# PrinceVictor/LWSNet

Measured on AMD Instinct MI355X. Metric: stereo pairs/sec @256x512 maxdisp=192 (stage-4), higher is better.
Workload: dtype f32; 1 GPU; BASELINE config 2: batch=1/GPU, 256x512 synthetic pair, maxdisplist=[24,5,5], all 4 stages; pairs_per_gpu=1, streams=1, parallelism=single GPU, weights=seeded synthetic (seed 7, calibrated BN), GPU_MAX_HW_QUEUES=4

## Files before the change

lwsnet_amd/csrc/lws_api.hip:

```cpp
#include <math.h>
#include <stdarg.h>
#include <stdio.h>
#include <string.h>

#include <algorithm>
#include <stdlib.h>

#include "lws_common.h"

namespace lws {

static thread_local char g_err[512] = "";
thread_local hipEvent_t tl_stop_event = nullptr;

void set_error(const char *fmt, ...)
{
    va_list ap;
    va_start(ap, fmt);
    vsnprintf(g_err, sizeof(g_err), fmt, ap);
    va_end(ap);
}

typedef std::map<std::string, std::vector<int64_t>> Spec;

// ... 701 lines not shown
                      "maxdisplist[%d] must be in 1..32 (got %d)", i, cfg->maxdisplist[i]);
    for (int i = 0; i < 3; ++i) {
        const int c3 = cfg->channels_3d * cfg->growth_rate[i];
        LWS_CHECK_ARG(c3 == 8 || c3 == 16 || c3 == 32,
                      "stage %d: channels_3d*growth_rate = %d is not supported by the gfx950 kernels (8, 16, 32)", i, c3);
    }
    LWS_CHECK_ARG(cfg->feature_fp16 == 0 || cfg->feature_fp16 == 1, "feature_fp16 must be 0 or 1 (got %d)", cfg->feature_fp16);
    LWS_CHECK_ARG(cfg->interp_align_mode == 0 || cfg->interp_align_mode == 1, "interp_align_mode must be 0 or 1 (got %d)",
                  cfg->interp_align_mode);
    lws_ctx *h = new (std::nothrow) lws_ctx();
    if (!h) {
        set_error("out of host memory");
        return LWS_ERR_NOMEM;
    }
    h->cfg = *cfg;
    h->spec = build_spec(*cfg);
    for (int i = 0; i < 3; ++i) h->stage[i].c3 = cfg->channels_3d * cfg->growth_rate[i];
    if (hipGetDevice(&h->device) != hipSuccess) h->device = -1;
    (void)hipGetLastError();
    *out = h;
    return LWS_OK;
}

static void apply_options(lws_ctx *h)
{
    for (int i = 0; i < 3; ++i) {
        h->stage[i].mid16_split = (h->opt.split_bf16 & 1) != 0;
        h->stage[i].mid8_split = (h->opt.split_bf16 & 2) != 0;
        h->stage[i].mid8_balance = h->mid8_balance;
        h->stage[i].cu_count = h->cu_count;
    }
    h->net2d.r2_first.form = (h->opt.split_bf16 & 4) ? 1 : 0;
}

static int *option_slot(lws_ctx *h, const char *name)
{
    struct { const char *name; int *slot; } tab[] = {{"fuse_first", &h->opt.fuse_first},
                                                     {"defer_upsample", &h->opt.defer_upsample},
                                                     {"side_streams", &h->opt.side_streams},
                                                     {"split_bf16", &h->opt.split_bf16},
                                                     {"ref_chunk_mb", &h->opt.ref_chunk_mb},
                                                     {"ref_pipe", &h->opt.ref_pipe},
                                                     {"warp_form", &h->opt.warp_form},
                                                     {"fuse_last1", &h->opt.fuse_last1},
                                                     {"fork2_after", &h->opt.fork2_after},
                                                     {"fuse_ref_last", &h->opt.fuse_ref_last},
                                                     {"device", &h->device}};
    for (auto &e : tab)
        if (strcmp(e.name, name) == 0) return e.slot;
    return nullptr;
}

int lws_set_option(lws_handle h, const char *name, int value)
{
    LWS_CHECK_ARG(h && name, "lws_set_option: null argument");
    int *slot = option_slot(h, name);
    LWS_CHECK_ARG(slot != nullptr, "lws_set_option: unknown option '%s'", name);
    if (strcmp(name, "split_bf16") == 0)
        LWS_CHECK_ARG(value >= 0 && value <= 7, "lws_set_option: split_bf16 is a bit mask in 0..7 (got %d)", value);
    else if (strcmp(name, "fuse_first") == 0)
        LWS_CHECK_ARG(value >= 0 && value <= 3, "lws_set_option: fuse_first is a bit mask in 0..3 (got %d)", value);
    else if (strcmp(name, "ref_pipe") == 0 || strcmp(name, "fuse_ref_last") == 0)
        LWS_CHECK_ARG(value >= -1 && value <= 1, "lws_set_option: %s is out of range (got %d)", name, value);
    else if (strcmp(name, "ref_chunk_mb") == 0)
        LWS_CHECK_ARG(value >= 0 && value <= 4096, "lws_set_option: ref_chunk_mb must be in 0..4096 (got %d)", value);
    else if (strcmp(name, "device") == 0) {
        LWS_CHECK_ARG(value >= 0, "lws_set_option: device must be >= 0 (got %d)", value);
        LWS_CHECK_ARG(h->params == nullptr && h->ws == nullptr && h->side == nullptr,
                      "lws_set_option: the device of a handle can only be changed before lws_finalize / lws_reserve "
                      "have allocated on device %d", h->device);
    }
    else if (strcmp(name, "fork2_after") == 0)
        LWS_CHECK_ARG(value >= -1 && value <= 16, "lws_set_option: fork2_after must be in -1..16 (got %d)", value);
    else
        LWS_CHECK_ARG(value == 0 || value == 1, "lws_set_option: %s must be 0 or 1 (got %d)", name, value);
    *slot = value;
    apply_options(h);
    return LWS_OK;
}

int lws_get_option(lws_handle h, const char *name, int *value)
{
    LWS_CHECK_ARG(h && name && value, "lws_get_option: null argument");
    int *slot = option_slot(h, name);
    LWS_CHECK_ARG(slot != nullptr, "lws_get_option: unknown option '%s'", name);
    *value = *slot;
    return LWS_OK;
}

int lws_profile_enable(lws_handle h, int class_mask)
{
    LWS_CHECK_ARG(h, "lws_profile_enable: null handle");
    prof_clear(h);
    h->prof_mask = h->prof_mask_cfg = (unsigned)class_mask;
    h->prof_every = 1;
    h->prof_calls = 0;
    return LWS_OK;
}

int lws_profile_sample(lws_handle h, int every_n)
{
    LWS_CHECK_ARG(h && every_n >= 1, "lws_profile_sample: every_n must be >= 1");
    h->prof_every = every_n;
    h->prof_calls = 0;
    return LWS_OK;
}

int lws_profile_read(lws_handle h, double *total_ms, int64_t *launches)
{
    LWS_CHECK_ARG(h && total_ms && launches, "lws_profile_read: null argument");
    LWS_CHECK_DEVICE(h, "lws_profile_read");
    for (int i = 0; i < LWS_KC_COUNT; ++i) {
        total_ms[i] = 0.0;
        launches[i] = 0;
    }
    for (lws_prof_rec &r : h->prof) {
        LWS_HIP(hipEventSynchronize(r.t1));
        float ms = 0.f;
        LWS_HIP(hipEventElapsedTime(&ms, r.t0, r.t1));
        total_ms[r.kc] += ms;
        launches[r.kc] += 1;
    }
    return LWS_OK;
}

int lws_profile_read_class(lws_handle h, int kernel_class, float *ms_out, int capacity, int *count)
{
    LWS_CHECK_ARG(h && count && (ms_out || capacity == 0) && capacity >= 0, "lws_profile_read_class: bad argument");
    LWS_CHECK_ARG(kernel_class >= 0 && kernel_class < LWS_KC_COUNT, "lws_profile_read_class: unknown kernel class %d", kernel_class);
    LWS_CHECK_DEVICE(h, "lws_profile_read_class");
    int n = 0;
    for (lws_prof_rec &r : h->prof) {
        if (r.kc != kernel_class) continue;
        if (n < capacity) {
            LWS_HIP(hipEventSynchronize(r.t1));
            float ms = 0.f;
            LWS_HIP(hipEventElapsedTime(&ms, r.t0, r.t1));
            ms_out[n] = ms;
        }
        ++n;
    }
    *count = n;
    return LWS_OK;
}

int lws_clock_stamp(lws_handle h, int enable)
{
    LWS_CHECK_ARG(h, "lws_clock_stamp: null handle");
    LWS_CHECK_DEVICE(h, "lws_clock_stamp");
    if (enable) {
        if (h->stage[0].c3 == 8) {
            set_error("lws_clock_stamp: stage 1 of this model has C3 = 8: no k_conv3d_mid16 launch to stamp");
            return LWS_ERR_STATE;
        }
        if (!h->clk_buf) LWS_HIP(hipMalloc(&h->clk_buf, kClockWgs * 4 * sizeof(unsigned long long)));
        LWS_HIP(hipMemset(h->clk_buf, 0, kClockWgs * 4 * sizeof(unsigned long long)));
    }
    h->stage[0].clk = enable ? h->clk_buf : nullptr;
    return LWS_OK;
}

int lws_clock_read(lws_handle h, double *ghz)
{
    LWS_CHECK_ARG(h && ghz, "lws_clock_read: null argument");
    LWS_CHECK_DEVICE(h, "lws_clock_read");
    if (!h->clk_buf) {
// ... 351 lines not shown
```

lwsnet_amd/csrc/lws_common.h:

```cpp
#pragma once
#include <hip/hip_runtime.h>
#include <hip/hip_ext.h>
#include <stdint.h>

#include <atomic>
#include <map>
#include <string>
#include <vector>

#include "lwsnet_hip.h"

namespace lws {

void set_error(const char *fmt, ...) __attribute__((format(printf, 1, 2)));

#define LWS_CHECK_ARG(cond, ...)                 \
    do {                                         \
        if (!(cond)) {                           \
            ::lws::set_error(__VA_ARGS__);       \
            return LWS_ERR_INVALID;              \
        }                                        \
    } while (0)

#define LWS_HIP(call)                                                                           \
// ... 169 lines not shown
struct lws_ctx {
    lws_config cfg;
    struct {
        int fuse_first = 3;
        int defer_upsample = 1;
        int side_streams = 1;
        int split_bf16 = 0;
        int ref_pipe = -1;
        int warp_form = 1;
        int fuse_last1 = 1;
        int fork2_after = -1;
        int fuse_ref_last = -1;
        int ref_chunk_mb = 72;
    } opt;
    unsigned prof_mask = 0;
    unsigned prof_mask_cfg = 0;
    int prof_every = 1;
    unsigned prof_calls = 0;
    std::vector<lws_prof_rec> prof;
    std::vector<hipEvent_t> evt_pool;
    int device = 0;
    int cu_count = 0;
    bool finalized = false;
    std::map<std::string, std::vector<float>> host;
    std::map<std::string, std::vector<int64_t>> shapes;
    std::map<std::string, std::vector<int64_t>> spec;
    float *params = nullptr;
    bool owns_params = true;
    size_t params_bytes = 0;
    lws::Stage3d stage[3];
    lws::Net2d net2d;
    bool have_2d = false;
    float *ws = nullptr;
    size_t ws_bytes = 0;
    int mid8_balance = 1;
    hipStream_t side = nullptr;
    hipEvent_t ev_fork = nullptr, ev_join = nullptr;
    hipEvent_t ev_feat[3] = {nullptr, nullptr, nullptr};
    hipEvent_t ev_fork2 = nullptr;
    unsigned long long *clk_buf = nullptr;
};

namespace lws {

struct StageMap {
    float *mem = nullptr;
    bool written = false;
    const float *low = nullptr;
    int h = 0, w = 0;
    StageMap *prev = nullptr;
};
int check_stage_map(const StageMap &m, bool nested, const char *who);

int launch_volume_l1_shift(const float *L, const float *R, float *cost, int B, int C, int h, int w, int D,
                           hipStream_t st, bool q16 = false);
int launch_volume_l1_warp(const float *L, const float *R, StageMap &prev, float *cost, float *wflow_out,
                          int B, int C, int h, int w, int H, int W, int m, hipStream_t st, bool q16 = false,
                          int form = 1,
                          float ioff = 0.5f);
int launch_softargmin(const float *cost, float *low, int B, int D, int h, int w, float start, hipStream_t st);
int launch_upsample_add(const float *low, const float *prev, float *out, int B, int h, int w, int H, int W,
                        hipStream_t st, float ioff = 0.5f);
int launch_softargmin_upsample(const float *cost, const float *prev, float *out, float *low_out, int B, int D, int h,
                               int w, int H, int W, float start, hipStream_t st, float ioff = 0.5f);

bool shift_first_can_fuse(const Stage3d &s, int C);
int launch_shift_first(const Stage3d &s, const float *L, const float *R, float *cost, float *act_out, int B, int C, int D,
                       int h, int w, hipStream_t st, bool q16);
int launch_conv3d_first(const Stage3d &s, const float *cost, float *act_out, int B, int D, int h, int w,
                        hipStream_t st);
int launch_conv3d_mid(const Stage3d &s, int layer, const float *act_in, float *act_out, int B, int D, int h,
                      int w, hipStream_t st, hipEvent_t e0 = nullptr, hipEvent_t e1 = nullptr);
int launch_conv3d_last(const Stage3d &s, const float *act_in, const float *cost_skip, float *cost_out, int B,
                       int D, int h, int w, hipStream_t st);

int launch_conv2d_nchw(const Conv2dLayer &l, const float *in, const float *res, float *out, int N, int H, int W,
                       hipStream_t st, const float *in2 = nullptr, int n1 = 0);
int conv2d_pair_groups(int layer);
void pack_pair_mfma(const float *w, int cin, float *out);
int launch_conv2d_pair(const Conv2dLayer &a, const Conv2dLayer &b, const float *in, const float *res, float *out, int N,
                       int H, int W, hipStream_t st, const float *in2 = nullptr, int n1 = 0);
int launch_ref_first(const float *in, int cin, const float *w, float *out, int B, int H, int W, hipStream_t st);
int launch_ref_dws(const RefDws &l, const float *in, float *out, int B, int H, int W, hipStream_t st);
bool ref_first_dws_can_fuse(const RefDws &l, int cin);
int launch_ref_first_dws(const RefDws &l, StageMap &in, int cin, const float *wfrag, float *out, int B, int H, int W,
                         hipStream_t st, float ioff = 0.5f);
int packed_first_mfma_floats(int cin);
void pack_first_mfma(const float *w , int cin, float *out);
int launch_ref_conv64(const RefConv64 &l, const float *inL, const float *inD, float *out, int B, int H, int W,
                      hipStream_t st);
int launch_ref_last(const float *in, const float *w, const float *pred3, float *out, int B, int H, int W, hipStream_t st);
bool ref_dws_last_can_fuse(const RefDws &l);
int launch_ref_dws_last(const RefDws &l, const float *in, const float *wlast, const float *pred3, float *out, int B, int H, int W,
                        hipStream_t st);
void pack_conv2d_mfma(const float *w, int cin, int ktaps, float *out);
size_t packed_conv64x_floats();
void pack_conv64_bf16x3(const float *w, float *out);

bool conv3d_last_can_fuse(const Stage3d &s, int D);
int launch_conv3d_last_softargmin(const Stage3d &s, const float *act_in, const float *cost_skip, float *cost_out,
                                  float *low, float start, int B, int D, int h, int w, hipStream_t st);

size_t packed_mid_weight_floats(int c3);
void pack_mid_weights(const float *w , int c3, float *out);
void pack_first8_weights(const float *w , float *out );
void pack_first16_weights(const float *w , int c3, float *out );

}
```

lwsnet_amd/csrc/lws_conv2d.hip:

```cpp
#include "lws_common.h"
#include "lws_device_math.h"

namespace lws {


LWS_DEFINE_STAMPS(conv2d)

__device__ __forceinline__ float bn_relu2(float x, float s, float t) { return fmaxf(fmaf(x, s, t), 0.0f); }
__device__ __forceinline__ float f4c(const float4 &v, int j) { return j == 0 ? v.x : j == 1 ? v.y : j == 2 ? v.z : v.w; }

template <int CIN, int COUT, bool TRANSPOSED>
__global__ __launch_bounds__(256) void k_conv2d_nchw(const float *__restrict__ in, const float *__restrict__ in2, int n1,
                                                     const float *__restrict__ wgt,
                                                     const float *__restrict__ bn_s, const float *__restrict__ bn_t,
                                                     const float *__restrict__ res, float *__restrict__ out, int H,
                                                     int W, int Ho, int Wo, int stride, int pad, int dil, int relu,
                                                     int RH, int RW, int RWp)
{
    constexpr int CPT = COUT / 4;
    extern __shared__ float sIn[];
    const int b = blockIdx.z;
    const int tid = threadIdx.x, tx = tid & 7, ty = (tid >> 3) & 7;
    const int wave_id = __builtin_amdgcn_readfirstlane(tid >> 6);
    const int co0 = wave_id * CPT;
// ... 420 lines not shown
}

int launch_conv2d_pair(const Conv2dLayer &a, const Conv2dLayer &b, const float *in, const float *res, float *out, int N,
                       int H, int W, hipStream_t st, const float *in2, int n1)
{
    if (a.transposed || b.transposed || b.stride != 1 || b.pad != b.dil || a.pad != a.dil || a.bn_s == nullptr ||
        b.cin != a.cout) {
        set_error("conv2d_pair: unsupported layer pair");
        return LWS_ERR_INVALID;
    }
    if (in2 == nullptr) {
        in2 = in;
        n1 = N;
    }
    const int HA = (H + 2 * a.pad - 2 * a.dil - 1) / a.stride + 1, WA = (W + 2 * a.pad - 2 * a.dil - 1) / a.stride + 1;
    if (a.cout == 16 && b.cout == 16 && a.stride == 2 && a.dil == 1 && b.dil == 1 && res == nullptr &&
        a.w_mfma != nullptr && b.w_mfma != nullptr && (a.cin == 8 || a.cin == 16)) {
        if (a.cin == 8) return conv2d_pair_mfma_launch<8>(a, b, in, in2, n1, out, N, H, W, HA, WA, st);
        return conv2d_pair_mfma_launch<16>(a, b, in, in2, n1, out, N, H, W, HA, WA, st);
    }
#define LWS_C2P(CI, CMID, CO, SA, DA, DB, NW)                                                             \
    if (a.cin == CI && a.cout == CMID && b.cout == CO && a.stride == SA && a.dil == DA && b.dil == DB)    \
        return conv2d_pair_launch<CI, CMID, CO, SA, DA, DB, NW>(a, b, in, in2, n1, res, out, N, H, W, HA, WA, st);
    LWS_C2P(3, 4, 8, 2, 2, 4, 4) LWS_C2P(8, 4, 8, 1, 2, 2, 4) LWS_C2P(8, 16, 16, 2, 1, 1, 16) LWS_C2P(16, 16, 16, 2, 1, 1, 16)
#undef LWS_C2P
    set_error("conv2d_pair: unsupported pair %d -> %d -> %d (stride %d, dilations %d, %d)", a.cin, a.cout, b.cout, a.stride,
              a.dil, b.dil);
    return LWS_ERR_INVALID;
}

template <int CIN>
__global__ __launch_bounds__(256) void k_ref_first(const float *__restrict__ in, const float *__restrict__ wgt,
                                                   float *__restrict__ out, int H, int W)
{
    __shared__ __attribute__((aligned(16))) float sW[9 * CIN * 32];
    for (int i = threadIdx.x; i < 9 * CIN * 32; i += 256) sW[i] = wgt[i];
    __syncthreads();
    const int64_t plane = (int64_t)H * W;
    const int64_t idx = (int64_t)blockIdx.x * 256 + threadIdx.x;
    const int64_t pix = idx >> 2;
    const int grp = (int)(idx & 3), b = blockIdx.y;
    if (pix >= plane) return;
    const int y = (int)(pix / W), x = (int)(pix % W);
    const float *inb = in + (int64_t)b * CIN * plane;
    float acc[8];
#pragma unroll
    for (int c = 0; c < 8; ++c) acc[c] = 0.0f;
#pragma unroll 3
    for (int tap = 0; tap < 9; ++tap) {
        const int kh = tap / 3, kw = tap - kh * 3;
        const int iy = y + kh - 1, ix = x + kw - 1;
        const bool ok = iy >= 0 && iy < H && ix >= 0 && ix < W;
#pragma unroll
        for (int ci = 0; ci < CIN; ++ci) {
            const float ld = inb[ok ? (int64_t)ci * plane + (int64_t)iy * W + ix : 0];
            const float v = ok ? ld : 0.0f;
            const float4 w0 = *reinterpret_cast<const float4 *>(&sW[(tap * CIN + ci) * 32 + grp * 8]);
            const float4 w1 = *reinterpret_cast<const float4 *>(&sW[(tap * CIN + ci) * 32 + grp * 8 + 4]);
            acc[0] = fmaf(v, w0.x, acc[0]);
            acc[1] = fmaf(v, w0.y, acc[1]);
            acc[2] = fmaf(v, w0.z, acc[2]);
            acc[3] = fmaf(v, w0.w, acc[3]);
            acc[4] = fmaf(v, w1.x, acc[4]);
            acc[5] = fmaf(v, w1.y, acc[5]);
            acc[6] = fmaf(v, w1.z, acc[6]);
            acc[7] = fmaf(v, w1.w, acc[7]);
        }
    }
    float4 *o = reinterpret_cast<float4 *>(out + ((int64_t)b * plane + pix) * 32 + grp * 8);
    o[0] = make_float4(acc[0], acc[1], acc[2], acc[3]);
    o[1] = make_float4(acc[4], acc[5], acc[6], acc[7]);
}

constexpr int RT_Y = 8, RT_X = 16;
constexpr int RH_Y = RT_Y + 2, RH_X = RT_X + 2;
constexpr int RVS = 32;

__device__ __forceinline__ int swz(int p, int grp) { return p * RVS + ((grp ^ (p & 7)) << 2); }

struct RefTile {
    int b, Y0, X0;
};

__device__ __forceinline__ RefTile ref_tile(int dil, int nbx, int nby, int tile_rows = RT_Y)
{
    int bid = blockIdx.x;
    const int d2 = dil * dil;
    const int phase = bid % d2;
    bid /= d2;
    const int bx = bid % nbx;
    bid /= nbx;
    const int by = bid % nby;
    RefTile t;
    t.b = bid / nby;
    t.Y0 = by * tile_rows * dil + phase / dil;
    t.X0 = bx * RT_X * dil + phase % dil;
    return t;
}

constexpr int DWS_SA = 186, DWS_SB = 130;

constexpr int DWS_FD = 2, DWS_FR = (RH_Y - 1) * DWS_FD + 3, DWS_FC = (RH_X - 1) * DWS_FD + 3;
static_assert(DWS_FR * DWS_FC <= 1024 && 3 * DWS_FR * DWS_FC <= 8 * DWS_SB * 4, "first-conv window must fit 4 loads/thread/plane and sB");

template <int CIN>
__device__ __forceinline__ void first_conv_mfma(const float *sImg, const float *__restrict__ wfrag,
                                                const float *__restrict__ bn_s, const float *__restrict__ bn_t, float4 *sA,
                                                int Y0, int X0, int H, int W, int lane, int wave)
{
    constexpr int WIN = DWS_FR * DWS_FC, K = 9 * CIN, J = (K + 3) / 4, NPX = RH_Y * RH_X, NTW = 3;
    static_assert(4 * NTW * 16 >= NPX, "three N-tiles per wave must cover the halo tile");
    const int n = lane & 15, g = lane >> 4;
    float a[2][J];
#pragma unroll
    for (int mt = 0; mt < 2; ++mt)
#pragma unroll
        for (int j = 0; j < J; ++j) a[mt][j] = wfrag[(mt * J + j) * 64 + lane];
    int koff[J];
#pragma unroll
    for (int j = 0; j < J; ++j) {
        const int k = 4 * j + g, tap = k / CIN, ci = k - tap * CIN, kh = tap / 3, kw = tap - kh * 3;
        koff[j] = k < K ? ci * WIN + kh * DWS_FC + kw : 0;
    }
    float4 s4[2], t4[2];
#pragma unroll
    for (int mt = 0; mt < 2; ++mt) {
        s4[mt] = *reinterpret_cast<const float4 *>(bn_s + (mt * 4 + g) * 4);
        t4[mt] = *reinterpret_cast<const float4 *>(bn_t + (mt * 4 + g) * 4);
    }
#pragma unroll
    for (int nt = 0; nt < NTW; ++nt) {
        const int hp = (wave * NTW + nt) * 16 + n;
        const int hy = hp / RH_X, hx = hp - hy * RH_X;
        const float *sp = sImg + (hp < NPX ? (hy * DWS_FD) * DWS_FC + hx * DWS_FD : 0);
        floatx4 acc[2] = {(floatx4){0.f, 0.f, 0.f, 0.f}, (floatx4){0.f, 0.f, 0.f, 0.f}};
#pragma unroll
        for (int j = 0; j < J; ++j) {
            const float b = sp[koff[j]];
#pragma unroll
            for (int mt = 0; mt < 2; ++mt) acc[mt] = __builtin_amdgcn_mfma_f32_16x16x4f32(a[mt][j], b, acc[mt], 0, 0, 0);
        }
        const int gy = Y0 + (hy - 1) * DWS_FD, gx = X0 + (hx - 1) * DWS_FD;
        const bool ok = hp < NPX && gy >= 0 && gy < H && gx >= 0 && gx < W;
#pragma unroll
        for (int mt = 0; mt < 2; ++mt) {
            float4 v = bn_relu4(make_float4(acc[mt][0], acc[mt][1], acc[mt][2], acc[mt][3]), s4[mt], t4[mt]);
            if (!ok) v = make_float4(0.f, 0.f, 0.f, 0.f);
            if (hp < NPX) sA[(mt * 4 + g) * DWS_SA + hp] = v;
        }
    }
}

template <int FIRST>
__global__ __launch_bounds__(256, 4) void k_ref_dws(const float *__restrict__ in, const float *__restrict__ wf,
                                                 const float *__restrict__ bn_s,
                                                 const float *__restrict__ bn_t, const float *dw,
                                                 const float4 *pwpk,
                                                 float *__restrict__ out, int H, int W, int dil, int nbx, int nby, int wt,
                                                 const float *__restrict__ plow, int ph, int pw, float *__restrict__ pmat,
                                                 float ioff)
{
    __shared__ float4 sA[8 * DWS_SA];
    __shared__ float4 sB[8 * DWS_SB];
    const int tid = threadIdx.x, lane = tid & 63, wave = tid >> 6;
    const RefTile t = ref_tile(dil, nbx, nby);
    LWS_STAMPK(5, 0);

    const int c4 = tid & 7;
    const float4 s4 = *reinterpret_cast<const float4 *>(bn_s + c4 * 4);
    const float4 t4 = *reinterpret_cast<const float4 *>(bn_t + c4 * 4);

    constexpr int NPX = RH_Y * RH_X, SITER = (NPX * 8 + 255) / 256;
    float4 c[SITER];
    bool okv[SITER];
    if (FIRST == 3) {
        float *sImg = reinterpret_cast<float *>(sB);
        constexpr int WIN = DWS_FR * DWS_FC, NLD = (3 * WIN + 255) / 256;
        const float *inb = in + (int64_t)t.b * 3 * H * W;
        const int gy0 = t.Y0 - DWS_FD - 1, gx0 = t.X0 - DWS_FD - 1;
        float iv[NLD];
#pragma unroll
        for (int k = 0; k < NLD; ++k) {
            const int r3 = tid + 256 * k;
            const int ci = r3 / WIN, r = r3 - ci * WIN;
            const int ry = r / DWS_FC, rx = r - ry * DWS_FC;
            const int gy = gy0 + ry, gx = gx0 + rx;
            const bool ok = r3 < 3 * WIN && gy >= 0 && gy < H && gx >= 0 && gx < W;
            const float ld = inb[ok ? (int64_t)ci * H * W + (int64_t)gy * W + gx : 0];
            iv[k] = ok ? ld : 0.0f;
        }
#pragma unroll
        for (int k = 0; k < NLD; ++k)
            if (tid + 256 * k < 3 * WIN) sImg[tid + 256 * k] = iv[k];
        __syncthreads();
        first_conv_mfma<3>(sImg, wf, bn_s, bn_t, sA, t.Y0, t.X0, H, W, lane, wave);
        __syncthreads();
    } else if (FIRST == 1) {
        float *sImg = reinterpret_cast<float *>(sB);
        DeferredMap dm{plow != nullptr ? plow + (int64_t)t.b * ph * pw : nullptr, in + (int64_t)t.b * H * W, ph, pw,
                       (float)H, 1.0f / (float)(ph > 0 ? ph : 1)};
        dm.off = ioff;
        const int gy0 = t.Y0 - DWS_FD - 1, gx0 = t.X0 - DWS_FD - 1;
        float iv[4];
        bool iok[4];
        int iys[4], ixs[4];
#pragma unroll
        for (int k = 0; k < 4; ++k) {
            const int r = tid + 256 * k;
            const int ry = r / DWS_FC, rx = r - ry * DWS_FC;
            const int gy = gy0 + ry, gx = gx0 + rx;
            iok[k] = r < DWS_FR * DWS_FC && gy >= 0 && gy < H && gx >= 0 && gx < W;
            iys[k] = iok[k] ? gy : 0;
            ixs[k] = iok[k] ? gx : 0;
        }
        deferred_at_n<4>(dm, iys, ixs, H, W, iv);
#pragma unroll
        for (int k = 0; k < 4; ++k)
            if (tid + 256 * k < DWS_FR * DWS_FC) sImg[tid + 256 * k] = iok[k] ? iv[k] : 0.0f;
        __syncthreads();
        if (pmat != nullptr && tid < RT_Y * RT_X) {
            const int ty = tid / RT_X, tx = tid - ty * RT_X;
            const int gy = t.Y0 + ty * DWS_FD, gx = t.X0 + tx * DWS_FD;
            if (gy < H && gx < W)
                pmat[(int64_t)t.b * H * W + (int64_t)gy * W + gx] = sImg[((ty + 1) * DWS_FD + 1) * DWS_FC + (tx + 1) * DWS_FD + 1];
        }
        first_conv_mfma<1>(sImg, wf, bn_s, bn_t, sA, t.Y0, t.X0, H, W, lane, wave);
        __syncthreads();
    } else {
        const float *inb = in + (int64_t)t.b * H * W * 32;
#pragma unroll
        for (int i = 0; i < SITER; ++i) {
            const int hp = (tid >> 3) + 32 * i;
            const int hy = hp / RH_X, hx = hp - hy * RH_X;
            const int gy = t.Y0 + (hy - 1) * dil, gx = t.X0 + (hx - 1) * dil;
            okv[i] = hp < NPX && gy >= 0 && gy < H && gx >= 0 && gx < W;
            const int off = okv[i] ? (gy * W + gx) * 32 + c4 * 4 : 0;
            c[i] = *reinterpret_cast<const float4 *>(inb + off);
        }
    }
    float4 aw[2][2];
#pragma unroll
    for (int q = 0; q < 2; ++q)
#pragma unroll
        for (int mt = 0; mt < 2; ++mt) aw[q][mt] = pwpk[(q * 2 + mt) * 64 + lane];
    float4 wd[9];
#pragma unroll
    for (int tap = 0; tap < 9; ++tap) wd[tap] = *reinterpret_cast<const float4 *>(dw + tap * 32 + c4 * 4);
    if (FIRST == 0) {
#pragma unroll
        for (int i = 0; i < SITER; ++i) {
            const int hp = (tid >> 3) + 32 * i;
            float4 v = bn_relu4(c[i], s4, t4);
            if (!okv[i]) v = make_float4(0.f, 0.f, 0.f, 0.f);
            if (hp < NPX) sA[c4 * DWS_SA + hp] = v;
        }
        __syncthreads();
    }
    LWS_STAMPK(5, 1);

    {
        const int q = c4 >> 2, a_ = c4 & 3;
        const int x = (tid >> 3) & 15, rg = tid >> 7;
        const float4 *src = sA + c4 * DWS_SA + (4 * rg) * RH_X + x;
        float4 acc[4];
#pragma unroll
        for (int j = 0; j < 4; ++j) acc[j] = make_float4(0.f, 0.f, 0.f, 0.f);
#pragma unroll
        for (int rr = 0; rr < 6; ++rr) {
            const float4 t0 = src[rr * RH_X], t1 = src[rr * RH_X + 1], t2 = src[rr * RH_X + 2];
#pragma unroll
            for (int j = 0; j < 4; ++j) {
                const int kh = rr - j;
                if (kh >= 0 && kh < 3) {
                    fma4(acc[j], t0, wd[kh * 3 + 0]);
                    fma4(acc[j], t1, wd[kh * 3 + 1]);
                    fma4(acc[j], t2, wd[kh * 3 + 2]);
                }
            }
        }
        float *dst = reinterpret_cast<float *>(sB + (4 * q) * DWS_SB + (4 * rg) * RT_X + x) + a_;
#pragma unroll
        for (int j = 0; j < 4; ++j) {
            dst[(0 * DWS_SB + RT_X * j) * 4] = acc[j].x;
            dst[(1 * DWS_SB + RT_X * j) * 4] = acc[j].y;
            dst[(2 * DWS_SB + RT_X * j) * 4] = acc[j].z;
            dst[(3 * DWS_SB + RT_X * j) * 4] = acc[j].w;
        }
    }
    __syncthreads();
    LWS_STAMPK(5, 2);

    const int n = lane & 15, g = lane >> 4;
    floatx4 acc[2][2];
#pragma unroll
    for (int r = 0; r < 2; ++r)
#pragma unroll
        for (int mt = 0; mt < 2; ++mt) acc[r][mt] = (floatx4){0.f, 0.f, 0.f, 0.f};
    float4 bv[2][2];
#pragma unroll
    for (int r = 0; r < 2; ++r)
#pragma unroll
        for (int q = 0; q < 2; ++q) bv[r][q] = sB[(4 * q + g) * DWS_SB + (2 * wave + r) * RT_X + n];
#pragma unroll
    for (int q = 0; q < 2; ++q)
#pragma unroll
        for (int j = 0; j < 4; ++j)
#pragma unroll
            for (int r = 0; r < 2; ++r)
#pragma unroll
                for (int mt = 0; mt < 2; ++mt)
                    acc[r][mt] = __builtin_amdgcn_mfma_f32_16x16x4f32(f4c(aw[q][mt], j), f4c(bv[r][q], j), acc[r][mt], 0, 0, 0);

    LWS_STAMPK(5, 3);
    float *outb = out + (int64_t)t.b * H * W * 32;
    const int gx = t.X0 + n * dil;
#pragma unroll
    for (int r = 0; r < 2; ++r) {
        const int gy = t.Y0 + (2 * wave + r) * dil;
        if (gy < H && gx < W) {
            float *o = outb + (gy * W + gx) * 32;
#pragma unroll
            for (int mt = 0; mt < 2; ++mt)
                store_act4(o + mt * 16 + 4 * g, make_float4(acc[r][mt][0], acc[r][mt][1], acc[r][mt][2], acc[r][mt][3]), wt);
        }
    }
}

template <int TY, int NW>
__global__ __launch_bounds__(64 * NW) void k_ref_conv64(const float *__restrict__ inL, const float *__restrict__ inD,
                                                    const float *__restrict__ bn_s, const float *__restrict__ bn_t,
                                                    const float4 *__restrict__ wpk,
                                                    float *__restrict__ out, int H, int W, int dil, int nbx, int nby, int wt)
{
    constexpr int HY = TY + 2, NPX = HY * RH_X, RW = TY / NW, NT = 64 * NW;
    static_assert(TY % NW == 0 && RW >= 1 && RW <= 4, "rows must split evenly over the waves");
    __shared__ __attribute__((aligned(16))) float sA[2 * NPX * RVS];
    const int tid = threadIdx.x, lane = tid & 63, wave = tid >> 6;
    const RefTile t = ref_tile(dil, nbx, nby, TY);
    const int n = lane & 15, g = lane >> 4;
    LWS_STAMPK(6, 0);

    constexpr int ITEMS = 2 * NPX * 2, SITER = (ITEMS + NT - 1) / NT;
    {
        float4 c[SITER][4];
        bool okv[SITER];
#pragma unroll
        for (int i = 0; i < SITER; ++i) {
            const int it = tid + i * NT;
            const int q = it & 1, hp = (it >> 1) % NPX, ten = (it >> 1) / NPX;
            const int hy = hp / RH_X, hx = hp % RH_X;
            const int gy = t.Y0 + (hy - 1) * dil, gx = t.X0 + (hx - 1) * dil;
            okv[i] = it < ITEMS && gy >= 0 && gy < H && gx >= 0 && gx < W;
            const float *base = (ten == 1 && it < ITEMS ? inD : inL) + (int64_t)t.b * H * W * 32;
            const float4 *src = reinterpret_cast<const float4 *>(base + (okv[i] ? ((int64_t)gy * W + gx) * 32 + q * 16 : 0));
#pragma unroll
            for (int k = 0; k < 4; ++k) c[i][k] = src[k];
        }
#pragma unroll
        for (int i = 0; i < SITER; ++i) {
            const int it = tid + i * NT;
            if (it < ITEMS) {
                const int q = it & 1, hp = (it >> 1) % NPX, ten = (it >> 1) / NPX;
                const float4 *sp = reinterpret_cast<const float4 *>(bn_s + ten * 32 + q * 16);
                const float4 *tp = reinterpret_cast<const float4 *>(bn_t + ten * 32 + q * 16);
                float4 a[4];
#pragma unroll
                for (int k = 0; k < 4; ++k) {
                    const float4 v = c[i][k], sc = sp[k], tt = tp[k];
                    a[k] = make_float4(bn_relu2(v.x, sc.x, tt.x), bn_relu2(v.y, sc.y, tt.y), bn_relu2(v.z, sc.z, tt.z),
                                       bn_relu2(v.w, sc.w, tt.w));
                    if (!okv[i]) a[k] = make_float4(0.f, 0.f, 0.f, 0.f);
                }
                float *img = sA + ten * NPX * RVS;
                *reinterpret_cast<float4 *>(&img[swz(hp, 4 * q + 0)]) = make_float4(a[0].x, a[1].x, a[2].x, a[3].x);
                *reinterpret_cast<float4 *>(&img[swz(hp, 4 * q + 1)]) = make_float4(a[0].y, a[1].y, a[2].y, a[3].y);
                *reinterpret_cast<float4 *>(&img[swz(hp, 4 * q + 2)]) = make_float4(a[0].z, a[1].z, a[2].z, a[3].z);
                *reinterpret_cast<float4 *>(&img[swz(hp, 4 * q + 3)]) = make_float4(a[0].w, a[1].w, a[2].w, a[3].w);
            }
        }
    }
    const float4 *wp = wpk + lane;
    float4 wbuf[2][4][2];
#pragma unroll
    for (int qq = 0; qq < 4; ++qq)
#pragma unroll
        for (int mt = 0; mt < 2; ++mt) wbuf[0][qq][mt] = wp[(qq * 2 + mt) * 64];
    __syncthreads();
    LWS_STAMPK(6, 1);

    floatx4 acc[RW][2];
#pragma unroll
    for (int r = 0; r < RW; ++r)
#pragma unroll
        for (int mt = 0; mt < 2; ++mt) acc[r][mt] = (floatx4){0.f, 0.f, 0.f, 0.f};
    auto frag = [&](int r, int tap, int qq) {
        const int hp = (RW * wave + r + tap / 3) * RH_X + n + tap % 3;
        return *reinterpret_cast<const float4 *>(&sA[(qq >> 1) * NPX * RVS + swz(hp, 4 * (qq & 1) + g)]);
    };
    float4 bbuf[2][RW];
#pragma unroll
    for (int r = 0; r < RW; ++r) bbuf[0][r] = frag(r, 0, 0);
#pragma unroll 1
    for (int tap = 0; tap < 9; ++tap) {
        const int tn = tap < 8 ? tap + 1 : 8;
#pragma unroll
        for (int qq = 0; qq < 4; ++qq) {
            float4 *bc = bbuf[qq & 1], *bn = bbuf[(qq & 1) ^ 1];
// ... 301 lines not shown
                dst[(2 * FL_SB) * 4] = acc.z;
                dst[(3 * FL_SB) * 4] = acc.w;
            }
        }
    }
    __syncthreads();

    {
        constexpr int NTW = FL_NT / 4;
        const int n = lane & 15, g = lane >> 4;
        floatx4 acc[NTW][2];
        float4 bv[NTW][2];
#pragma unroll
        for (int r = 0; r < NTW; ++r) {
#pragma unroll
            for (int mt = 0; mt < 2; ++mt) acc[r][mt] = (floatx4){0.f, 0.f, 0.f, 0.f};
#pragma unroll
            for (int q = 0; q < 2; ++q) bv[r][q] = sB[(4 * q + g) * FL_SB + (wave * NTW + r) * 16 + n];
        }
#pragma unroll
        for (int q = 0; q < 2; ++q)
#pragma unroll
            for (int j = 0; j < 4; ++j)
#pragma unroll
                for (int r = 0; r < NTW; ++r)
#pragma unroll
                    for (int mt = 0; mt < 2; ++mt)
                        acc[r][mt] = __builtin_amdgcn_mfma_f32_16x16x4f32(f4c(aw[q][mt], j), f4c(bv[r][q], j), acc[r][mt], 0, 0, 0);
#pragma unroll
        for (int r = 0; r < NTW; ++r) {
            const int p = (wave * NTW + r) * 16 + n;
            if (p < FL_NM) {
                const int my = p / FL_MX, mx = p - my * FL_MX;
                const int gy = t.Y0 + my - 1, gx = t.X0 + mx - 1;
                const bool ok = gy >= 0 && gy < H && gx >= 0 && gx < W;
#pragma unroll
                for (int mt = 0; mt < 2; ++mt)
                    sC[(4 * mt + g) * FL_SC + p] = ok ? make_float4(acc[r][mt][0], acc[r][mt][1], acc[r][mt][2], acc[r][mt][3])
                                                      : make_float4(0.f, 0.f, 0.f, 0.f);
            }
        }
    }
    __syncthreads();

    if (tid < RT_Y * RT_X) {
        const int ty = tid >> 4, tx = tid & 15;
        const int y = t.Y0 + ty, x = t.X0 + tx;
        const bool live = y < H && x < W;
        const int64_t o = ((int64_t)t.b * H + (live ? y : 0)) * W + (live ? x : 0);
        const float skip = pred3[o];
        float acc = 0.0f;
#pragma unroll
        for (int kh = 0; kh < 3; ++kh)
#pragma unroll
            for (int kw = 0; kw < 3; ++kw) {
                const float4 *p = sC + (ty + kh) * FL_MX + tx + kw;
                const float *w = wlast + (kh * 3 + kw) * 32;
#pragma unroll
                for (int g8 = 0; g8 < 8; ++g8) {
                    const float4 a = p[g8 * FL_SC];
                    acc = fmaf(a.x, w[g8 * 4 + 0], acc);
                    acc = fmaf(a.y, w[g8 * 4 + 1], acc);
                    acc = fmaf(a.z, w[g8 * 4 + 2], acc);
                    acc = fmaf(a.w, w[g8 * 4 + 3], acc);
                }
            }
        if (live) out[o] = acc + skip;
    }
}

int launch_ref_first(const float *in, int cin, const float *w, float *out, int B, int H, int W, hipStream_t st)
{
    dim3 grid((unsigned)(((int64_t)H * W * 4 + 255) / 256), B), block(256);
    if (cin == 3) hipLaunchKernelGGL(k_ref_first<3>, grid, block, 0, st, in, w, out, H, W);
    else if (cin == 1) hipLaunchKernelGGL(k_ref_first<1>, grid, block, 0, st, in, w, out, H, W);
    else {
        set_error("ref_first: unsupported cin %d", cin);
        return LWS_ERR_INVALID;
    }
    LWS_LAUNCH_CHECK();
    return LWS_OK;
}

int launch_ref_dws(const RefDws &l, const float *in, float *out, int B, int H, int W, hipStream_t st)
{
    const int nbx = cdiv(W, RT_X * l.dil), nby = cdiv(H, RT_Y * l.dil);
    dim3 grid(nbx * nby * l.dil * l.dil * B), block(256);
    hipLaunchKernelGGL(k_ref_dws<0>, grid, block, 0, st, in, (const float *)nullptr, l.bn_s, l.bn_t, l.dw,
                       reinterpret_cast<const float4 *>(l.pw), out, H, W, l.dil, nbx, nby,
                       use_wt_stores((size_t)B * H * W * 128), (const float *)nullptr, 0, 0, (float *)nullptr, 0.5f);
    LWS_LAUNCH_CHECK();
    return LWS_OK;
}

bool ref_first_dws_can_fuse(const RefDws &l, int cin) { return (cin == 1 || cin == 3) && l.dil == DWS_FD; }

int packed_first_mfma_floats(int cin) { return 2 * ((9 * cin + 3) / 4) * 64; }
void pack_first_mfma(const float *w, int cin, float *out)
{
    const int K = 9 * cin, J = (K + 3) / 4;
    for (int mt = 0; mt < 2; ++mt)
        for (int j = 0; j < J; ++j)
            for (int lane = 0; lane < 64; ++lane) {
                const int m = lane & 15, g = lane >> 4, k = 4 * j + g, tap = k / cin, ci = k % cin;
                out[(mt * J + j) * 64 + lane] = k < K ? w[((16 * mt + m) * cin + ci) * 9 + tap] : 0.0f;
            }
}

int launch_ref_first_dws(const RefDws &l, StageMap &in, int cin, const float *wfrag, float *out, int B, int H, int W,
                         hipStream_t st, float ioff)
{
    if (!ref_first_dws_can_fuse(l, cin)) {
        set_error("ref_first_dws: cin %d / dilation %d unsupported", cin, l.dil);
        return LWS_ERR_INVALID;
    }
    if (cin != 1 && !in.written) {
        set_error("ref_first_dws: only the one-channel (disparity) input can be a deferred map");
        return LWS_ERR_INVALID;
    }
    const int rc = check_stage_map(in, false, "ref_first_dws");
    if (rc) return rc;
    const bool def = !in.written;
    const int nbx = cdiv(W, RT_X * l.dil), nby = cdiv(H, RT_Y * l.dil);
    dim3 grid(nbx * nby * l.dil * l.dil * B), block(256);
    const int wt = use_wt_stores((size_t)B * H * W * 128);
    const float4 *pw4 = reinterpret_cast<const float4 *>(l.pw);
    const float *img = def ? in.prev->mem : in.mem;
    if (cin == 3)
        hipLaunchKernelGGL(k_ref_dws<3>, grid, block, 0, st, img, wfrag, l.bn_s, l.bn_t, l.dw, pw4, out, H, W, l.dil, nbx, nby, wt,
                           (const float *)nullptr, 0, 0, (float *)nullptr, ioff);
    else
        hipLaunchKernelGGL(k_ref_dws<1>, grid, block, 0, st, img, wfrag, l.bn_s, l.bn_t, l.dw, pw4, out, H, W, l.dil, nbx, nby, wt,
                           def ? in.low : nullptr, def ? in.h : 0, def ? in.w : 0, def ? in.mem : nullptr, ioff);
    LWS_LAUNCH_CHECK();
    in.written = true;
    return LWS_OK;
}

int launch_ref_conv64(const RefConv64 &l, const float *inL, const float *inD, float *out, int B, int H, int W,
                      hipStream_t st)
{
    const int dil = 8;
    if (l.form == 1) {
        using Cfg = Conv64xCfg<8, 4>;
        static std::atomic<uint64_t> attr_done{0};
        const int rc_ = ensure_dyn_lds(attr_done, reinterpret_cast<const void *>(&k_ref_conv64x<8, 4>), Cfg::LDS_BYTES);
        if (rc_ != LWS_OK) return rc_;
        const int nbx = cdiv(W, RT_X * dil), nby = cdiv(H, 8 * dil);
        dim3 grid(nbx * nby * dil * dil * B), block(Cfg::NT);
        hipLaunchKernelGGL((k_ref_conv64x<8, 4>), grid, block, Cfg::LDS_BYTES, st, inL, inD, l.bn_s, l.bn_t,
                           reinterpret_cast<const uint4 *>(l.wx), out, H, W, dil, nbx, nby,
                           use_wt_stores((size_t)B * H * W * 128));
        LWS_LAUNCH_CHECK();
        return LWS_OK;
    }
#define LWS_C64(TYv, NWv)                                                                                          \
    {                                                                                                               \
        const int nbx = cdiv(W, RT_X * dil), nby = cdiv(H, TYv * dil);                                              \
        dim3 grid(nbx * nby * dil * dil * B), block(64 * NWv);                                                      \
        hipLaunchKernelGGL((k_ref_conv64<TYv, NWv>), grid, block, 0, st, inL, inD, l.bn_s, l.bn_t,                   \
                           reinterpret_cast<const float4 *>(l.w), out, H, W, dil, nbx, nby,                         \
                           use_wt_stores((size_t)B * H * W * 128));                                                 \
    }
    LWS_C64(8, 4);
#undef LWS_C64
    LWS_LAUNCH_CHECK();
    return LWS_OK;
}

bool ref_dws_last_can_fuse(const RefDws &l) { return l.dil == 1; }

int launch_ref_dws_last(const RefDws &l, const float *in, const float *wlast, const float *pred3, float *out, int B, int H, int W,
                        hipStream_t st)
{
    if (!ref_dws_last_can_fuse(l)) {
        set_error("ref_dws_last: dilation %d unsupported", l.dil);
        return LWS_ERR_INVALID;
    }
    const int nbx = cdiv(W, RT_X), nby = cdiv(H, RT_Y);
    dim3 grid(nbx * nby * B), block(256);
    hipLaunchKernelGGL(k_ref_dws_last, grid, block, 0, st, in, l.bn_s, l.bn_t, l.dw, reinterpret_cast<const float4 *>(l.pw), wlast,
                       pred3, out, H, W, nbx, nby);
    LWS_LAUNCH_CHECK();
    return LWS_OK;
}

int launch_ref_last(const float *in, const float *w, const float *pred3, float *out, int B, int H, int W, hipStream_t st)
{
    dim3 grid(cdiv(W, LAST_TX), cdiv(H, LAST_TY), B), block(256);
    hipLaunchKernelGGL(k_ref_last, grid, block, 0, st, in, w, pred3, out, H, W);
    LWS_LAUNCH_CHECK();
    return LWS_OK;
}

void pack_conv2d_mfma(const float *w, int cin, int ktaps, float *out)
{
    const int Q = cin / 16;
    for (int tap = 0; tap < ktaps; ++tap)
        for (int q = 0; q < Q; ++q)
            for (int mt = 0; mt < 2; ++mt)
                for (int lane = 0; lane < 64; ++lane)
                    for (int j = 0; j < 4; ++j) {
                        const int m = lane & 15, g = lane >> 4;
                        const int co = 16 * mt + m, ci = 16 * q + 4 * j + g;
                        out[((((size_t)tap * Q + q) * 2 + mt) * 64 + lane) * 4 + j] = w[((size_t)co * cin + ci) * ktaps + tap];
                    }
}

size_t packed_conv64x_floats() { return (size_t)20 * 2 * 3 * 64 * 4; }
void pack_conv64_bf16x3(const float *w, float *out)
{
    uint16_t *ox = reinterpret_cast<uint16_t *>(out);
    for (int step = 0; step < 20; ++step)
        for (int mt = 0; mt < 2; ++mt)
            for (int lane = 0; lane < 64; ++lane)
                for (int j = 0; j < 8; ++j) {
// ... 9 lines not shown
```

Baseline: 2132 pairs/s.

## Pipeline ref_dws tiles with async global-to-LDS double-buffered loads

```diff
diff --git a/lwsnet_amd/csrc/lws_api.hip b/lwsnet_amd/csrc/lws_api.hip
--- a/lwsnet_amd/csrc/lws_api.hip
+++ b/lwsnet_amd/csrc/lws_api.hip
@@ -807,6 +807,10 @@
 int lws_get_option(lws_handle h, const char *name, int *value)
 {
     LWS_CHECK_ARG(h && name && value, "lws_get_option: null argument");
+    if (strcmp(name, "ref_dws_pipe_launches") == 0 || strcmp(name, "ref_dws_tile_launches") == 0) {
+        *value = ref_dws_launch_count(strcmp(name, "ref_dws_pipe_launches") == 0);
+        return LWS_OK;
+    }
     int *slot = option_slot(h, name);
     LWS_CHECK_ARG(slot != nullptr, "lws_get_option: unknown option '%s'", name);
     *value = *slot;
diff --git a/lwsnet_amd/csrc/lws_common.h b/lwsnet_amd/csrc/lws_common.h
--- a/lwsnet_amd/csrc/lws_common.h
+++ b/lwsnet_amd/csrc/lws_common.h
@@ -275,6 +275,7 @@
                        int H, int W, hipStream_t st, const float *in2 = nullptr, int n1 = 0);
 int launch_ref_first(const float *in, int cin, const float *w, float *out, int B, int H, int W, hipStream_t st);
 int launch_ref_dws(const RefDws &l, const float *in, float *out, int B, int H, int W, hipStream_t st);
+int ref_dws_launch_count(int pipelined);
 bool ref_first_dws_can_fuse(const RefDws &l, int cin);
 int launch_ref_first_dws(const RefDws &l, StageMap &in, int cin, const float *wfrag, float *out, int B, int H, int W,
                          hipStream_t st, float ioff = 0.5f);
diff --git a/lwsnet_amd/csrc/lws_conv2d.hip b/lwsnet_amd/csrc/lws_conv2d.hip
--- a/lwsnet_amd/csrc/lws_conv2d.hip
+++ b/lwsnet_amd/csrc/lws_conv2d.hip
@@ -526,9 +526,8 @@
     int b, Y0, X0;
 };
 
-__device__ __forceinline__ RefTile ref_tile(int dil, int nbx, int nby, int tile_rows = RT_Y)
-{
-    int bid = blockIdx.x;
+__device__ __forceinline__ RefTile ref_tile_at(int bid, int dil, int nbx, int nby, int tile_rows = RT_Y)
+{
     const int d2 = dil * dil;
     const int phase = bid % d2;
     bid /= d2;
@@ -541,6 +540,10 @@
     t.X0 = bx * RT_X * dil + phase % dil;
     return t;
 }
+__device__ __forceinline__ RefTile ref_tile(int dil, int nbx, int nby, int tile_rows = RT_Y)
+{
+    return ref_tile_at(blockIdx.x, dil, nbx, nby, tile_rows);
+}
 
 constexpr int DWS_SA = 186, DWS_SB = 130;
 
@@ -595,24 +598,62 @@
     }
 }
 
-template <int FIRST>
-__global__ __launch_bounds__(256, 4) void k_ref_dws(const float *__restrict__ in, const float *__restrict__ wf,
+constexpr int DWS_RAW = 23 * 64;
+static_assert(DWS_RAW >= RH_Y * RH_X * 8 && (2 * DWS_RAW + 8 * DWS_SB) * 16 <= 64 * 1024, "k_ref_dws<0, true> LDS images");
+
+__device__ __forceinline__ void glds16(const float *g, unsigned lds_byte)
+{
+#if defined(__HIP_DEVICE_COMPILE__)
+    unsigned keep;
+    asm volatile("s_mov_b32 %0, m0\n\ts_mov_b32 m0, %2\n\ts_nop 0\n\tglobal_load_lds_dwordx4 %1, off\n\ts_mov_b32 m0, %0"
+                 : "=&s"(keep)
+                 : "v"(g), "s"(lds_byte)
+                 : "memory");
+#endif
+}
+
+template <int FIRST, bool PIPE = false>
+__global__ __launch_bounds__(256, PIPE ? 2 : 4) void k_ref_dws(const float *__restrict__ in, const float *__restrict__ wf,
                                                  const float *__restrict__ bn_s,
                                                  const float *__restrict__ bn_t, const float *dw,
                                                  const float4 *pwpk,
                                                  float *__restrict__ out, int H, int W, int dil, int nbx, int nby, int wt,
                                                  const float *__restrict__ plow, int ph, int pw, float *__restrict__ pmat,
-                                                 float ioff)
-{
-    __shared__ float4 sA[8 * DWS_SA];
+                                                 float ioff, int tpw, int ntiles)
+{
+    static_assert(!PIPE || FIRST == 0, "the pipelined form exists for the plain block only");
+    __shared__ float4 sA[PIPE ? 2 * DWS_RAW : 8 * DWS_SA];
     __shared__ float4 sB[8 * DWS_SB];
     const int tid = threadIdx.x, lane = tid & 63, wave = tid >> 6;
-    const RefTile t = ref_tile(dil, nbx, nby);
+    const int tile0 = PIPE ? blockIdx.x * tpw : blockIdx.x;
+    const int ntl = PIPE ? min(tpw, ntiles - tile0) : 1;
+    RefTile t = ref_tile_at(tile0, dil, nbx, nby);
     LWS_STAMPK(5, 0);
 
+    constexpr int NPC = (DWS_RAW / 64 + 3) / 4;
+    auto piece_off = [&](const RefTile &tt, int k, bool &ok) {
+        const int hp = (4 * k + wave) * 8 + (lane >> 3);
+        const int hy = hp / RH_X, hx = hp - hy * RH_X;
+        const int gy = tt.Y0 + (hy - 1) * dil, gx = tt.X0 + (hx - 1) * dil;
+        ok = hp < RH_Y * RH_X && gy >= 0 && gy < H && gx >= 0 && gx < W;
+        return ok ? (gy * W + gx) * 32 + (lane & 7) * 4 : 0;
+    };
+    auto issue_tile = [&](const RefTile &tt, int buf) {
+        const float *inb = in + (int64_t)tt.b * H * W * 32;
+        const unsigned lds0 = (unsigned)(size_t)(__attribute__((address_space(3))) float4 *)(sA + buf * DWS_RAW);
+#pragma unroll
+        for (int k = 0; k < NPC; ++k)
+            if (4 * k + wave < DWS_RAW / 64) {
+                bool ok;
+                const int off = piece_off(tt, k, ok);
+                glds16(inb + off, __builtin_amdgcn_readfirstlane(lds0 + (4 * k + wave) * 1024));
+            }
+    };
+    if (PIPE) issue_tile(t, 0);
+
     const int c4 = tid & 7;
-    const float4 s4 = *reinterpret_cast<const float4 *>(bn_s + c4 * 4);
-    const float4 t4 = *reinterpret_cast<const float4 *>(bn_t + c4 * 4);
+    float4 s4 = *reinterpret_cast<const float4 *>(bn_s + c4 * 4);
+    float4 t4 = *reinterpret_cast<const float4 *>(bn_t + c4 * 4);
 
     constexpr int NPX = RH_Y * RH_X, SITER = (NPX * 8 + 255) / 256;
     float4 c[SITER];
@@ -670,7 +711,7 @@
         }
         first_conv_mfma<1>(sImg, wf, bn_s, bn_t, sA, t.Y0, t.X0, H, W, lane, wave);
         __syncthreads();
-    } else {
+    } else if (!PIPE) {
         const float *inb = in + (int64_t)t.b * H * W * 32;
 #pragma unroll
         for (int i = 0; i < SITER; ++i) {
@@ -690,7 +731,7 @@
     float4 wd[9];
 #pragma unroll
     for (int tap = 0; tap < 9; ++tap) wd[tap] = *reinterpret_cast<const float4 *>(dw + tap * 32 + c4 * 4);
-    if (FIRST == 0) {
+    if (FIRST == 0 && !PIPE) {
 #pragma unroll
         for (int i = 0; i < SITER; ++i) {
             const int hp = (tid >> 3) + 32 * i;
@@ -700,73 +741,123 @@
         }
         __syncthreads();
     }
-    LWS_STAMPK(5, 1);
-
-    {
-        const int q = c4 >> 2, a_ = c4 & 3;
-        const int x = (tid >> 3) & 15, rg = tid >> 7;
-        const float4 *src = sA + c4 * DWS_SA + (4 * rg) * RH_X + x;
-        float4 acc[4];
-#pragma unroll
-        for (int j = 0; j < 4; ++j) acc[j] = make_float4(0.f, 0.f, 0.f, 0.f);
-#pragma unroll
-        for (int rr = 0; rr < 6; ++rr) {
-            const float4 t0 = src[rr * RH_X], t1 = src[rr * RH_X + 1], t2 = src[rr * RH_X + 2];
-#pragma unroll
-            for (int j = 0; j < 4; ++j) {
-                const int kh = rr - j;
-                if (kh >= 0 && kh < 3) {
-                    fma4(acc[j], t0, wd[kh * 3 + 0]);
-                    fma4(acc[j], t1, wd[kh * 3 + 1]);
-                    fma4(acc[j], t2, wd[kh * 3 + 2]);
-                }
-            }
-        }
-        float *dst = reinterpret_cast<float *>(sB + (4 * q) * DWS_SB + (4 * rg) * RT_X + x) + a_;
-#pragma unroll
-        for (int j = 0; j < 4; ++j) {
-            dst[(0 * DWS_SB + RT_X * j) * 4] = acc[j].x;
-            dst[(1 * DWS_SB + RT_X * j) * 4] = acc[j].y;
-            dst[(2 * DWS_SB + RT_X * j) * 4] = acc[j].z;
-            dst[(3 * DWS_SB + RT_X * j) * 4] = acc[j].w;
-        }
-    }
-    __syncthreads();
-    LWS_STAMPK(5, 2);
-
+    if (PIPE) {
+        auto pin4 = [](float4 &v) { asm volatile("" : "+v"(v.x), "+v"(v.y), "+v"(v.z), "+v"(v.w)); };
+        pin4(s4), pin4(t4);
+#pragma unroll
+        for (int q = 0; q < 2; ++q)
+#pragma unroll
+            for (int mt = 0; mt < 2; ++mt) pin4(aw[q][mt]);
+#pragma unroll
+        for (int tap = 0; tap < 9; ++tap) pin4(wd[tap]);
+    }
     const int n = lane & 15, g = lane >> 4;
     floatx4 acc[2][2];
-#pragma unroll
-    for (int r = 0; r < 2; ++r)
-#pragma unroll
-        for (int mt = 0; mt < 2; ++mt) acc[r][mt] = (floatx4){0.f, 0.f, 0.f, 0.f};
-    float4 bv[2][2];
-#pragma unroll
-    for (int r = 0; r < 2; ++r)
-#pragma unroll
-        for (int q = 0; q < 2; ++q) bv[r][q] = sB[(4 * q + g) * DWS_SB + (2 * wave + r) * RT_X + n];
-#pragma unroll
-    for (int q = 0; q < 2; ++q)
-#pragma unroll
-        for (int j = 0; j < 4; ++j)
-#pragma unroll
-            for (int r = 0; r < 2; ++r)
+    auto store_tile = [&](const RefTile &tt) {
+        float *outb = out + (int64_t)tt.b * H * W * 32;
+        const int gx = tt.X0 + n * dil;
+#pragma unroll
+        for (int r = 0; r < 2; ++r) {
+            const int gy = tt.Y0 + (2 * wave + r) * dil;
+            if (gy < H && gx < W) {
+                float *o = outb + (gy * W + gx) * 32;
 #pragma unroll
                 for (int mt = 0; mt < 2; ++mt)
-                    acc[r][mt] = __builtin_amdgcn_mfma_f32_16x16x4f32(f4c(aw[q][mt], j), f4c(bv[r][q], j), acc[r][mt], 0, 0, 0);
-
-    LWS_STAMPK(5, 3);
-    float *outb = out + (int64_t)t.b * H * W * 32;
-    const int gx = t.X0 + n * dil;
-#pragma unroll
-    for (int r = 0; r < 2; ++r) {
-        const int gy = t.Y0 + (2 * wave + r) * dil;
-        if (gy < H && gx < W) {
-            float *o = outb + (gy * W + gx) * 32;
-#pragma unroll
-            for (int mt = 0; mt < 2; ++mt)
-                store_act4(o + mt * 16 + 4 * g, make_float4(acc[r][mt][0], acc[r][mt][1], acc[r][mt][2], acc[r][mt][3]), wt);
-        }
+                    store_act4(o + mt * 16 + 4 * g, make_float4(acc[r][mt][0], acc[r][mt][1], acc[r][mt][2], acc[r][mt][3]), wt);
+            }
+        }
+    };
+
+    RefTile tprev = t, tnext = t;
+    for (int i = 0;; ++i) {
+        const float4 *img = sA;
+        constexpr int PS = PIPE ? 8 : 1;
+        if (PIPE) {
+            if (i < ntl) {
+                __builtin_amdgcn_s_waitcnt(0x0f70);
+                asm volatile("" ::: "memory");
+            }
+            if (i == 0) LWS_STAMPK(5, 1);
+            if (i == 1) LWS_STAMPK(5, 4);
+            if (i + 1 < ntl) {
+                tnext = ref_tile_at(tile0 + i + 1, dil, nbx, nby);
+                issue_tile(tnext, (i + 1) & 1);
+            }
+            if (i > 0) store_tile(tprev);
+            if (i == ntl) break;
+            float4 *raw = sA + (i & 1) * DWS_RAW;
+#pragma unroll
+            for (int k = 0; k < NPC; ++k)
+                if (4 * k + wave < DWS_RAW / 64) {
+                    bool ok;
+                    piece_off(t, k, ok);
+                    float4 v = bn_relu4(raw[(4 * k + wave) * 64 + lane], s4, t4);
+                    if (!ok) v = make_float4(0.f, 0.f, 0.f, 0.f);
+                    raw[(4 * k + wave) * 64 + lane] = v;
+                }
+            __syncthreads();
+            img = raw;
+        } else {
+            LWS_STAMPK(5, 1);
+        }
+
+        {
+            const int q = c4 >> 2, a_ = c4 & 3;
+            const int x = (tid >> 3) & 15, rg = tid >> 7;
+            const float4 *src = PIPE ? img + ((4 * rg) * RH_X + x) * PS + c4 : img + c4 * DWS_SA + (4 * rg) * RH_X + x;
+            float4 dacc[4];
+#pragma unroll
+            for (int j = 0; j < 4; ++j) dacc[j] = make_float4(0.f, 0.f, 0.f, 0.f);
+#pragma unroll
+            for (int rr = 0; rr < 6; ++rr) {
+                const float4 t0 = src[(rr * RH_X) * PS], t1 = src[(rr * RH_X + 1) * PS], t2 = src[(rr * RH_X + 2) * PS];
+#pragma unroll
+                for (int j = 0; j < 4; ++j) {
+                    const int kh = rr - j;
+                    if (kh >= 0 && kh < 3) {
+                        fma4(dacc[j], t0, wd[kh * 3 + 0]);
+                        fma4(dacc[j], t1, wd[kh * 3 + 1]);
+                        fma4(dacc[j], t2, wd[kh * 3 + 2]);
+                    }
+                }
+            }
+            float *dst = reinterpret_cast<float *>(sB + (4 * q) * DWS_SB + (4 * rg) * RT_X + x) + a_;
+#pragma unroll
+            for (int j = 0; j < 4; ++j) {
+                dst[(0 * DWS_SB + RT_X * j) * 4] = dacc[j].x;
+                dst[(1 * DWS_SB + RT_X * j) * 4] = dacc[j].y;
+                dst[(2 * DWS_SB + RT_X * j) * 4] = dacc[j].z;
+                dst[(3 * DWS_SB + RT_X * j) * 4] = dacc[j].w;
+            }
+        }
+        __syncthreads();
+        if (i == 0) LWS_STAMPK(5, 2);
+
+#pragma unroll
+        for (int r = 0; r < 2; ++r)
+#pragma unroll
+            for (int mt = 0; mt < 2; ++mt) acc[r][mt] = (floatx4){0.f, 0.f, 0.f, 0.f};
+        float4 bv[2][2];
+#pragma unroll
+        for (int r = 0; r < 2; ++r)
+#pragma unroll
+            for (int q = 0; q < 2; ++q) bv[r][q] = sB[(4 * q + g) * DWS_SB + (2 * wave + r) * RT_X + n];
+#pragma unroll
+        for (int q = 0; q < 2; ++q)
+#pragma unroll
+            for (int j = 0; j < 4; ++j)
+#pragma unroll
+                for (int r = 0; r < 2; ++r)
+#pragma unroll
+                    for (int mt = 0; mt < 2; ++mt)
+                        acc[r][mt] = __builtin_amdgcn_mfma_f32_16x16x4f32(f4c(aw[q][mt], j), f4c(bv[r][q], j), acc[r][mt], 0, 0, 0);
+        if (i == 0) LWS_STAMPK(5, 3);
+        if (!PIPE) {
+            store_tile(t);
+            break;
+        }
+        tprev = t;
+        t = tnext;
     }
 }
 
@@ -1234,14 +1325,40 @@
     return LWS_OK;
 }
 
+#ifndef LWS_REF_DWS_PIPE_MAX
+#define LWS_REF_DWS_PIPE_MAX 4
+#endif
+static std::atomic<int> g_ref_dws_launches[2];
+int ref_dws_launch_count(int pipelined) { return g_ref_dws_launches[pipelined ? 1 : 0].load(std::memory_order_relaxed); }
+
+static int ref_dws_tiles_per_wg(int tiles)
+{
+    static const int cus = [] {
+        int dev = 0, n = 0;
+        if (hipGetDevice(&dev) != hipSuccess || hipDeviceGetAttribute(&n, hipDeviceAttributeMultiprocessorCount, dev) != hipSuccess)
+            n = 0;
+        return n > 0 ? n : 256;
+    }();
+    const int tpw = cdiv(tiles, 2 * cus);
+    return tpw >= 2 && tpw <= LWS_REF_DWS_PIPE_MAX ? tpw : 0;
+}
+
 int launch_ref_dws(const RefDws &l, const float *in, float *out, int B, int H, int W, hipStream_t st)
 {
     const int nbx = cdiv(W, RT_X * l.dil), nby = cdiv(H, RT_Y * l.dil);
-    dim3 grid(nbx * nby * l.dil * l.dil * B), block(256);
-    hipLaunchKernelGGL(k_ref_dws<0>, grid, block, 0, st, in, (const float *)nullptr, l.bn_s, l.bn_t, l.dw,
-                       reinterpret_cast<const float4 *>(l.pw), out, H, W, l.dil, nbx, nby,
-                       use_wt_stores((size_t)B * H * W * 128), (const float *)nullptr, 0, 0, (float *)nullptr, 0.5f);
+    const int tiles = nbx * nby * l.dil * l.dil * B, tpw = ref_dws_tiles_per_wg(tiles);
+    dim3 block(256);
+    const int wt = use_wt_stores((size_t)B * H * W * 128);
+    const float4 *pw4 = reinterpret_cast<const float4 *>(l.pw);
+    if (tpw > 0)
+        hipLaunchKernelGGL((k_ref_dws<0, true>), dim3(cdiv(tiles, tpw)), block, 0, st, in, (const float *)nullptr, l.bn_s, l.bn_t,
+                           l.dw, pw4, out, H, W, l.dil, nbx, nby, wt, (const float *)nullptr, 0, 0, (float *)nullptr, 0.5f, tpw,
+                           tiles);
+    else
+        hipLaunchKernelGGL(k_ref_dws<0>, dim3(tiles), block, 0, st, in, (const float *)nullptr, l.bn_s, l.bn_t, l.dw, pw4, out, H,
+                           W, l.dil, nbx, nby, wt, (const float *)nullptr, 0, 0, (float *)nullptr, 0.5f, 1, tiles);
     LWS_LAUNCH_CHECK();
+    g_ref_dws_launches[tpw > 0 ? 1 : 0].fetch_add(1, std::memory_order_relaxed);
     return LWS_OK;
 }
 
@@ -1280,10 +1397,10 @@
     const float *img = def ? in.prev->mem : in.mem;
     if (cin == 3)
         hipLaunchKernelGGL(k_ref_dws<3>, grid, block, 0, st, img, wfrag, l.bn_s, l.bn_t, l.dw, pw4, out, H, W, l.dil, nbx, nby, wt,
-                           (const float *)nullptr, 0, 0, (float *)nullptr, ioff);
+                           (const float *)nullptr, 0, 0, (float *)nullptr, ioff, 1, 0);
     else
         hipLaunchKernelGGL(k_ref_dws<1>, grid, block, 0, st, img, wfrag, l.bn_s, l.bn_t, l.dw, pw4, out, H, W, l.dil, nbx, nby, wt,
-                           def ? in.low : nullptr, def ? in.h : 0, def ? in.w : 0, def ? in.mem : nullptr, ioff);
+                           def ? in.low : nullptr, def ? in.h : 0, def ? in.w : 0, def ? in.mem : nullptr, ioff, 1, 0);
     LWS_LAUNCH_CHECK();
     in.written = true;
     return LWS_OK;
```

Measured after the change: 2075 pairs/s. -2.7%, worse.
